# yuriyvnv/speech_transcript_embeddings

Hardware: AMD Instinct MI355X
Metric: audio–text pairs/sec (whole node), 10s@16kHz + 64-tok, 1/2/4/8 MI355X (higher is better)
Workload: dtype bf16; 1 GPU; c2: global batch 64 = 1 GPU x 1 micro-batch(es) of 64 pairs, each pair 10s@16kHz audio + 64-tok clean + 64-tok corrupt; w2v-bert-2.0 Conformer 24L + XLM-R-base 12L, 3+3 unfrozen; GPU fbank -> fwd -> InfoNCE -> bwd -> allreduce -> clip+AdamW; global_batch=64, local_batch=64, micro_batch=64, accumulation_steps=1, seq_len_audio_frames=499, seq_len_text=64, parallelism=dp1

## Files before the change

profiles/attn_probe.py:

```python
import argparse
import json
import os
import sys

import torch

sys.path.insert(0, os.path.dirname(os.path.dirname(os.path.abspath(__file__))))


def main():
    ap = argparse.ArgumentParser()
    ap.add_argument("--batch", type=int, default=64)
    ap.add_argument("--frames", type=int, default=499)
    ap.add_argument("--heads", type=int, default=16)
    ap.add_argument("--iters", type=int, default=20)
    ap.add_argument("--no-bwd", action="store_true")
    ap.add_argument("--no-split", action="store_true", help="forward without the O_lo (hi + lo P) product")
    a = ap.parse_args()
    from speech_transcript_embeddings_amd import ops
    B, T, H = a.batch, a.frames, a.heads
    D = 64 * H
    M = B * T
    g = torch.Generator(device="cuda").manual_seed(0)
    qkv = torch.randn(M, 3 * D, device="cuda", generator=g) * 0.6
    qkv[:, 2 * D:] += torch.randn(B, 1, D, device="cuda", generator=g).expand(B, T, D).reshape(M, D)
    qkv = qkv.bfloat16()
    q, k, v = qkv[:, :D], qkv[:, D:2 * D], qkv[:, 2 * D:]
    mask = torch.ones(B, T, dtype=torch.int32, device="cuda")
    for b in range(0, B, 4):
        mask[b, T - 1 - (b % 37):] = 0
    mask = mask.reshape(-1).contiguous()
    E = (torch.randn(73, 64, device="cuda", generator=g) * 0.3).bfloat16()
    o = torch.empty(M, D, device="cuda", dtype=torch.bfloat16)
    o_lo = torch.empty_like(o)
    lse = torch.empty(B * H * T, device="cuda")
    do = (torch.randn(M, D, device="cuda", generator=g)).bfloat16()
    dqkv = torch.empty(M, 3 * D, device="cuda", dtype=torch.bfloat16)
    delta = torch.empty(B * H * T, device="cuda")
    dE = torch.zeros(73, 64, device="cuda")
    gwork = torch.empty(B * H * T * 80, device="cuda")

    def fwd():
        ops.attention_fwd(q, k, v, B=B, T=T, H=H, o=o, lse=lse, key_mask=mask, rel_E=E, scale=0.125,
                          o_lo=None if a.no_split else o_lo)

    def bwd():
        ops.attention_bwd(q, k, v, o, lse, do, dqkv[:, :D], dqkv[:, D:2 * D], dqkv[:, 2 * D:], B=B, T=T, H=H,
                          delta=delta, key_mask=mask, rel_E=E, scale=0.125, dE=dE, gwork=gwork, o_lo=o_lo)

    fwd()
    if not a.no_bwd:
        bwd()
    torch.cuda.synchronize()
    res = {}
    for name, fn in (("fwd", fwd),) + (() if a.no_bwd else (("bwd", bwd),)):
        e0, e1 = torch.cuda.Event(enable_timing=True), torch.cuda.Event(enable_timing=True)
        e0.record()
        for _ in range(a.iters):
            fn()
        e1.record()
        torch.cuda.synchronize()
        res[name + "_us"] = round(e0.elapsed_time(e1) * 1e3 / a.iters, 1)
    fl = 4.0 * B * H * T * T * 64
    fl_rel = 2.0 * B * H * T * 73 * 64
    res["fwd_tflops"] = round((fl + fl_rel) / res["fwd_us"] / 1e6, 1)
    if "bwd_us" in res:
        res["bwd_tflops"] = round((2.5 * fl + 2 * fl_rel) / res["bwd_us"] / 1e6, 1)
    res["shape"] = {"B": B, "T": T, "H": H}
    print(json.dumps(res), flush=True)


if __name__ == "__main__":
    main()
```

speech_transcript_embeddings_amd/csrc/attention.hip:

```cpp
#include <type_traits>
#include "common.h"
#include "../../include/ste.h"

#ifndef STE_ABLATE
#define STE_ABLATE 0
#endif

namespace {

constexpr int HD = 64;
constexpr int TQ = 64;
constexpr int TK = 64;
constexpr int NT = 256;
constexpr int TILE = TK * HD * 2;
constexpr int NREL = 80;
constexpr float NEG_MASK = -3.4028234663852886e38f;

STE_DEV int swz(int row, int chunk) { return row * 128 + ((chunk ^ (row & 7)) << 4); }

STE_DEV int med3i(int d, int lo, int hi) {
  int r;
  asm("v_med3_i32 %0, %1, %2, %3" : "=v"(r) : "v"(d), "v"(lo), "v"(hi));
  return r;
}

STE_DEV void tile_ld(bf16x8 (&r)[2], const bf16* base, int64_t ld, int bT, int row0, int T, int tid) {
#pragma unroll
  for (int i = 0; i < 2; ++i) {
    int c = tid + NT * i, row = c >> 3, ch = c & 7;
    if (row0 + row < T) r[i] = *reinterpret_cast<const bf16x8*>(base + (int64_t)(bT + row0 + row) * ld + ch * 8);
    else r[i] = bf16x8{};
  }
}
STE_DEV void tile_st(char* t, const bf16x8 (&r)[2], int tid) {
#pragma unroll
  for (int i = 0; i < 2; ++i) {
    int c = tid + NT * i;
    *reinterpret_cast<bf16x8*>(t + swz(c >> 3, c & 7)) = r[i];
  }
}
STE_DEV bf16x8 frag_kc(const char* t, int rb, int s, int lane) {
  int r = rb + (lane & 15);
  return *reinterpret_cast<const bf16x8*>(t + swz(r, s * 4 + (lane >> 4)));
}
STE_DEV int tr_off(int row, int quad) { return row * 128 + ((((quad >> 1) ^ (row & 7))) << 4) + ((quad & 1) << 3); }
STE_DEV bf16x8 frag_tr(const char* t, int cb, int u, int lane) {
  int g = lane >> 4, li = lane & 15, q = li >> 2, p = li & 3;
  int r0 = 32 * u + 4 * g + q;
  int quad = (cb >> 2) + p;
  return join_tr(ds_read_tr16(t + tr_off(r0, quad)), ds_read_tr16(t + tr_off(r0 + 16, quad)));
}
STE_DEV bf16x8 pack_acc(f32x4 a, f32x4 b) {
  bf16x8 v;
  v[0] = (bf16)a[0]; v[1] = (bf16)a[1]; v[2] = (bf16)a[2]; v[3] = (bf16)a[3];
  v[4] = (bf16)b[0]; v[5] = (bf16)b[1]; v[6] = (bf16)b[2]; v[7] = (bf16)b[3];
  return v;
}

typedef float f32x2 __attribute__((ext_vector_type(2)));

STE_DEV bf16x8 pack_acc_lo(f32x4 a, f32x4 b, bf16x8 hi) {
  typedef unsigned u32x4 __attribute__((ext_vector_type(4)));
  const u32x4 hu = __builtin_bit_cast(u32x4, hi);
  const f32x4 x[2] = {a, b};
  bf16x8 v;
#pragma unroll
  for (int w = 0; w < 4; ++w) {
    const f32x2 h = {__builtin_bit_cast(float, hu[w] << 16), __builtin_bit_cast(float, hu[w] & 0xffff0000u)};
    const f32x2 d = f32x2{x[w >> 1][2 * (w & 1)], x[w >> 1][2 * (w & 1) + 1]} - h;
    v[2 * w] = (bf16)d[0];
    v[2 * w + 1] = (bf16)d[1];
  }
  return v;
}

STE_DEV void stage_E(char* sE, const bf16* E, int nrel, int rows, int tid) {
  for (int c = tid; c < rows * 8; c += NT) {
    int row = c >> 3, ch = c & 7;
    bf16x8 v = bf16x8{};
    if (row < nrel) v = *reinterpret_cast<const bf16x8*>(E + row * HD + ch * 8);
    *reinterpret_cast<bf16x8*>(sE + swz(row, ch)) = v;
  }
}
STE_DEV void build_qe(float* qe, const char* sE, const bf16x8 (&qf)[2], int lane) {
  const int g = lane >> 4, li = lane & 15;
#pragma unroll
  for (int jt = 0; jt < NREL / 16; ++jt) {
    f32x4 acc = {0.f, 0.f, 0.f, 0.f};
#pragma unroll
    for (int s = 0; s < 2; ++s) acc = mfma16(frag_kc(sE, jt * 16, s, lane), qf[s], acc);
#pragma unroll
    for (int r = 0; r < 4; ++r) qe[li * NREL + jt * 16 + 4 * g + r] = acc[r];
  }
}

STE_DEV float key_flag(const int32_t* mask, int bT, int key, int T) {
  if (key >= T) return -1.f;
  return (mask == nullptr || mask[bT + key] != 0) ? 1.f : 0.f;
}

STE_DEV void tile_of_block(int T, int H, int& tile, int& h, int& b) {
  const int ntile = (T + 63) / 64;
  const int id = xcd_remap(blockIdx.x, gridDim.x);
  tile = id % ntile;
  const int bh = id / ntile;
  h = bh % H;
  b = bh / H;
}

template <bool REL, bool DROP>
__global__ __launch_bounds__(NT, 2) void attn_fwd_kernel(ste_attn_args a) {
  extern __shared__ __attribute__((aligned(16))) char sm[];
  char* sK = sm;
  char* sV = sm + 2 * TILE;
  char* sE = sm + 4 * TILE;
  float* sQE = reinterpret_cast<float*>(sE + NREL * 128);
  float* sMask = sQE + 4 * 16 * NREL;

  const int tid = threadIdx.x, lane = tid & 63, w = tid >> 6, g = lane >> 4, li = lane & 15;
  int tile, h, b;
  tile_of_block(a.T, a.H, tile, h, b);
  const int T = a.T, H = a.H, bT = b * T;
  const int q0 = tile * TQ + w * 16, myq = q0 + li;
  const bf16* Qb = (const bf16*)a.q + h * HD;
  const bf16* Kb = (const bf16*)a.k + h * HD;
  const bf16* Vb = (const bf16*)a.v + h * HD;
  const int left = a.rel_left, right = a.rel_right, nrel = left + right + 1;

  bf16x8 qf[2];
#pragma unroll
  for (int s = 0; s < 2; ++s)
    qf[s] = myq < T ? *reinterpret_cast<const bf16x8*>(Qb + (int64_t)(bT + myq) * a.ldq + 32 * s + 8 * g) : bf16x8{};

  float* qe = sQE + w * 16 * NREL;
  float qe_lo = 0.f, qe_hi = 0.f;
  if (REL) {
    stage_E(sE, (const bf16*)a.rel_E, nrel, NREL, tid);
    __syncthreads();
    build_qe(qe, sE, qf, lane);
    __builtin_amdgcn_s_waitcnt(0xc07f);
    __builtin_amdgcn_wave_barrier();
    qe_lo = qe[li * NREL];
    qe_hi = qe[li * NREL + nrel - 1];
  }

  const uint32_t thresh = (uint32_t)(a.drop_p * 4294967296.0);
  const float inv_keep = DROP ? 1.0f / (1.0f - a.drop_p) : 1.0f;
  const uint64_t drow = ((uint64_t)(b * H + h) * T + myq) * (uint64_t)T;
  const bool split = a.o_lo != nullptr;

  float m = -INFINITY, l = 0.f;
  f32x4 o[4];
#pragma unroll
  for (int i = 0; i < 4; ++i) o[i] = f32x4{0.f, 0.f, 0.f, 0.f};

  const int nkt = (T + TK - 1) / TK;
  bf16x8 rk[2], rv[2];
  tile_ld(rk, Kb, a.ldk, bT, 0, T, tid);
  tile_ld(rv, Vb, a.ldv, bT, 0, T, tid);
  tile_st(sK, rk, tid);
  tile_st(sV, rv, tid);
  if (tid < 64) sMask[tid] = key_flag(a.key_mask, bT, tid, T);
  __syncthreads();

  for (int kt = 0; kt < nkt; ++kt) {
    const int cur = kt & 1, kb = kt * TK;
    const bool more = kt + 1 < nkt;
    float mk_next = 0.f;
    if (more) {
      tile_ld(rk, Kb, a.ldk, bT, kb + TK, T, tid);
      tile_ld(rv, Vb, a.ldv, bT, kb + TK, T, tid);
      if (tid < 64) mk_next = key_flag(a.key_mask, bT, kb + TK + tid, T);
    }
    const char* tK = sK + cur * TILE;
    const char* tV = sV + cur * TILE;
    const float* mk = sMask + cur * 64;

    f32x4 s[4];
#pragma unroll
    for (int t = 0; t < 4; ++t) {
      s[t] = f32x4{0.f, 0.f, 0.f, 0.f};
#pragma unroll
      for (int ss = 0; ss < 2; ++ss) s[t] = mfma16(frag_kc(tK, t * 16, ss, lane), qf[ss], s[t]);
    }
    const bool all_lo = (kb + TK - 1) - q0 <= -left;
    const bool all_hi = kb - (q0 + 15) >= right;
    float tmax = -INFINITY;
#pragma unroll
    for (int t = 0; t < 4; ++t)
#pragma unroll
      for (int r = 0; r < 4; ++r) {
        const int kl = 16 * t + 4 * g + r;
        float bias = 0.f;
        if (REL) {
          if (all_lo) bias = qe_lo;
          else if (all_hi) bias = qe_hi;
          else {
            int d = kb + kl - myq;
            d = med3i(d, -left, right);
            bias = qe[li * NREL + d + left];
          }
        }
        float v = (s[t][r] + bias) * a.scale;
        const float f = mk[kl];
        v = f > 0.5f ? v : (f < -0.5f ? -INFINITY : NEG_MASK);
        s[t][r] = v;
        tmax = fmaxf(tmax, v);
      }
    tmax = fmaxf(tmax, __shfl_xor(tmax, 16, 64));
    tmax = fmaxf(tmax, __shfl_xor(tmax, 32, 64));
    const float mnew = fmaxf(m, tmax);
    const float alpha = (mnew == -INFINITY) ? 1.f : __expf(m - mnew);
    float psum = 0.f;
#pragma unroll
    for (int t = 0; t < 4; ++t)
#pragma unroll
      for (int r = 0; r < 4; ++r) {
        float p = (mnew == -INFINITY) ? 0.f : __expf(s[t][r] - mnew);
        psum += p;
        if (DROP) p *= drop_scale(a.seed, drow + (uint64_t)(kb + 16 * t + 4 * g + r), thresh, inv_keep);
        s[t][r] = p;
      }
    psum += __shfl_xor(psum, 16, 64);
    psum += __shfl_xor(psum, 32, 64);
    l = l * alpha + psum;
    m = mnew;
#pragma unroll
    for (int dt = 0; dt < 4; ++dt) o[dt] *= alpha;
#pragma unroll
    for (int u = 0; u < 2; ++u) {
      const bf16x8 pb = pack_acc(s[2 * u], s[2 * u + 1]);
#pragma unroll
      for (int dt = 0; dt < 4; ++dt) o[dt] = mfma16(frag_tr(tV, dt * 16, u, lane), pb, o[dt]);
      if (split) {
        const bf16x8 pl = pack_acc_lo(s[2 * u], s[2 * u + 1], pb);
#pragma unroll
        for (int dt = 0; dt < 4; ++dt) o[dt] = mfma16(frag_tr(tV, dt * 16, u, lane), pl, o[dt]);
      }
    }
    if (more) {
      tile_st(sK + (cur ^ 1) * TILE, rk, tid);
      tile_st(sV + (cur ^ 1) * TILE, rv, tid);
      if (tid < 64) sMask[(cur ^ 1) * 64 + tid] = mk_next;
    }
    __syncthreads();
  }
  if (myq < T) {
    const bool zrow = a.zero_masked_rows && m == NEG_MASK;
    const float inv_l = zrow ? 0.f : 1.0f / l;
    bf16* O = (bf16*)a.o + (int64_t)(bT + myq) * a.ldo + h * HD;
    if (a.o_lo) {
      bf16* Ol = (bf16*)a.o_lo + (int64_t)(bT + myq) * a.ldolo + h * HD;
#pragma unroll
      for (int dt = 0; dt < 4; ++dt) store_bf16x4_split(O + 16 * dt + 4 * g, Ol + 16 * dt + 4 * g, o[dt] * inv_l);
    } else {
#pragma unroll
      for (int dt = 0; dt < 4; ++dt) store_bf16x4(O + 16 * dt + 4 * g, o[dt] * inv_l);
    }
    if (g == 0) a.lse[(int64_t)(b * H + h) * T + myq] = m == NEG_MASK ? (zrow ? INFINITY : -INFINITY) : m + logf(l);
  }
}
// ... 1008 lines not shown
    }
#pragma unroll
    for (int gq = 0; gq < 2; ++gq) {
      const int q0g = qw + 16 * gq, myq = q0g + li;
      float* row = tb + (16 * gq + li) * GT3 + left;
      const bool all_lo = nrel == 1 || (kb + TK - 1) - q0g <= -left;
      const bool all_hi = kb - (q0g + 15) >= right;
      const bool band = !(all_lo || all_hi);
      if (!band) {
        const float cb = all_lo ? blo[gq] : bhi[gq];
#pragma unroll
        for (int t = 0; t < 4; ++t)
#pragma unroll
          for (int r = 0; r < 4; ++r) sc[gq][t][r] = __builtin_amdgcn_exp2f(fmaf(sc[gq][t][r], c2, cb));
      } else {
#pragma unroll
        for (int t = 0; t < 4; ++t)
#pragma unroll
          for (int r = 0; r < 4; ++r) {
            int d = kb + 16 * t + 4 * g + r - myq;
            d = med3i(d, -left, right);
            sc[gq][t][r] = __builtin_amdgcn_exp2f(fmaf(sc[gq][t][r] + row[d], c2, nl2[gq]));
          }
      }
      if (!all_valid) {
#pragma unroll
        for (int t = 0; t < 4; ++t)
#pragma unroll
          for (int r = 0; r < 4; ++r) {
            const int bit = 4 * t + r;
            const float fill = ((inp >> bit) & 1u) ? pm[gq] : 0.f;
            sc[gq][t][r] = ((okp >> bit) & 1u) ? sc[gq][t][r] : fill;
          }
      }
      float bsum = 0.f;
#pragma unroll
      for (int t = 0; t < 4; ++t)
#pragma unroll
        for (int r = 0; r < 4; ++r) {
          const float ds = sc[gq][t][r] * (dp[gq][t][r] - dl[gq]);
          sc[gq][t][r] = ds;
          bsum += ds;
        }
      if (!band) {
        if (all_lo) glo[gq] += bsum; else ghi[gq] += bsum;
      } else {
        float* spare = row + (GT3 - 1 - left);
#pragma unroll
        for (int t = 0; t < 4; ++t)
#pragma unroll
          for (int r = 0; r < 4; ++r) {
            const int d = kb + 16 * t + 4 * g + r - myq;
            const bool lo = d <= -left, hi = d >= right;
            glo[gq] += lo ? sc[gq][t][r] : 0.f;
            ghi[gq] += hi ? sc[gq][t][r] : 0.f;
            *((lo || hi) ? spare : row + d) = sc[gq][t][r];
          }
      }
    }
    asm volatile("s_waitcnt lgkmcnt(0)" ::: "memory");
    __builtin_amdgcn_sched_barrier(0);
#pragma unroll
    for (int gq = 0; gq < 2; ++gq)
#pragma unroll
      for (int u = 0; u < 2; ++u) {
        const bf16x8 pb = pack_acc(sc[gq][2 * u], sc[gq][2 * u + 1]);
#pragma unroll
        for (int dt = 0; dt < 4; ++dt) dq[gq][dt] = mfma16(ktr[dt][u], pb, dq[gq][dt]);
      }
    if (kt + 1 < nkt) {
      asm volatile("s_waitcnt vmcnt(0)" ::: "memory");
      __builtin_amdgcn_s_barrier();
      if (kt + 2 < nkt) issue(kt + 2);
    }
  }
  if (nkt > 1) issue_E(sm + (nkt & 1) * KV);
  const int kend = nkt * TK;
#pragma unroll
  for (int gq = 0; gq < 2; ++gq) {
    glo[gq] = rowsum4(glo[gq]);
    ghi[gq] = rowsum4(ghi[gq]);
    const int myq = qw + 16 * gq + li;
    float* row = tb + (16 * gq + li) * GT3;
    for (int j = 1 + g; j < nrel - 1; j += 4) {
      const int k = myq + j - left;
      if (k < 0 || k >= kend) row[j] = 0.f;
    }
    if (g == 1) row[GT3 - 1] = 0.f;
    if (g == 0) {
      row[0] = glo[gq];
      if (nrel > 1) row[nrel - 1] = ghi[gq];
    }
  }
  asm volatile("s_waitcnt vmcnt(0)" ::: "memory");
  __syncthreads();
  const char* sE = sm + (nkt & 1) * KV;
#pragma unroll
  for (int gq = 0; gq < 2; ++gq) {
    const float* row = tb + (16 * gq + li) * GT3;
#pragma unroll
    for (int u = 0; u < 2; ++u) {
      const f32x4 g0 = *reinterpret_cast<const f32x4*>(row + 32 * u + 4 * g);
      const f32x4 g1 = *reinterpret_cast<const f32x4*>(row + 32 * u + 16 + 4 * g);
      const bf16x8 pb = pack_acc(g0, g1);
#pragma unroll
      for (int dt = 0; dt < 4; ++dt) dq[gq][dt] = mfma16(frag_tr(sE, dt * 16, u, lane), pb, dq[gq][dt]);
    }
    const f32x4 gt4 = *reinterpret_cast<const f32x4*>(row + 64 + 4 * g);
    bf16x4 gb;
    gb[0] = (bf16)gt4[0]; gb[1] = (bf16)gt4[1]; gb[2] = (bf16)gt4[2]; gb[3] = (bf16)gt4[3];
    const int q = li >> 2, pq = li & 3;
#pragma unroll
    for (int dt = 0; dt < 4; ++dt) {
      const s16x4 ea = ds_read_tr16(sE + tr_off(64 + 4 * g + q, dt * 4 + pq));
      dq[gq][dt] = __builtin_amdgcn_mfma_f32_16x16x16bf16_1k(ea, __builtin_bit_cast(s16x4, gb), dq[gq][dt], 0, 0, 0);
    }
  }
#pragma unroll
  for (int gq = 0; gq < 2; ++gq) {
    const int myq = qw + 16 * gq + li;
    if (myq >= T) continue;
    const int64_t rowid = (int64_t)(b * H + h) * T + myq;
    const float* row = tb + (16 * gq + li) * GT3;
    if (a.dE) {
      float* G = a.gwork + rowid * NREL;
#pragma unroll
      for (int c = 0; c < NREL / 16; ++c) {
        const int j = c * 16 + 4 * g;
        *reinterpret_cast<f32x4*>(G + j) = *reinterpret_cast<const f32x4*>(row + j);
      }
    }
    bf16* dQ = (bf16*)a.dq + (int64_t)(bT + myq) * a.lddq + h * HD;
#pragma unroll
    for (int dt = 0; dt < 4; ++dt) store_bf16x4(dQ + 16 * dt + 4 * g, dq[gq][dt] * a.scale);
  }
}

namespace rel2 {
constexpr int KB = 128;
constexpr int QD = 2 * TILE + 512;
constexpr int KV_E_OFF = 2 * QD;
constexpr int KV_QE_OFF = KV_E_OFF + NREL * 128;
constexpr int QE3 = NREL + 4;
constexpr int KV_EDGE3_OFF = KV_QE_OFF + 64 * QE3 * 4;
constexpr int DKV3_LDS = KV_EDGE3_OFF + 512;
}

__global__ __launch_bounds__(NT, 2) void attn_bwd_dkv_rel3_kernel(ste_attn_args a) {
  using namespace rel2;
  extern __shared__ __attribute__((aligned(16))) char sm[];
  const int tid = threadIdx.x, lane = tid & 63, g = lane >> 4, li = lane & 15;
  const int w = __builtin_amdgcn_readfirstlane(tid >> 6);
  const int T = a.T, H = a.H;
  const int ntile = (T + KB - 1) / KB;
  const int id = xcd_remap(blockIdx.x, gridDim.x);
  const int tile = id % ntile, bh = id / ntile, h = bh % H, b = bh / H, bT = b * T;
  const int left = a.rel_left, right = a.rel_right, nrel = left + right + 1;
  const bf16* Qb = (const bf16*)a.q + h * HD;
  const bf16* Kb = (const bf16*)a.k + h * HD;
  const bf16* Vb = (const bf16*)a.v + h * HD;
  const bf16* dOb = (const bf16*)a.dout + h * HD;
  const int kb0 = tile * KB, k0w = kb0 + w * 32;
  const int64_t rowbase = (int64_t)(b * H + h) * T;
  const float c2 = a.scale * LOG2E;

  bf16x8 kf[2][2], vf[2][2];
  bool kmask[2];
#pragma unroll
  for (int gk = 0; gk < 2; ++gk) {
    const int key = k0w + 16 * gk + li;
    const bool kv = key < T;
    kmask[gk] = kv && a.key_mask != nullptr && a.key_mask[bT + key] == 0;
#pragma unroll
    for (int s = 0; s < 2; ++s) {
      kf[gk][s] = kv ? *reinterpret_cast<const bf16x8*>(Kb + (int64_t)(bT + key) * a.ldk + 32 * s + 8 * g) : bf16x8{};
      vf[gk][s] = kv ? *reinterpret_cast<const bf16x8*>(Vb + (int64_t)(bT + key) * a.ldv + 32 * s + 8 * g) : bf16x8{};
    }
  }
  const bool any_masked = __ballot(kmask[0] || kmask[1]) != 0;
  char* sE = sm + KV_E_OFF;
  float* qet3 = reinterpret_cast<float*>(sm + KV_QE_OFF);
  float* elo = reinterpret_cast<float*>(sm + KV_EDGE3_OFF);
  float* ehi = elo + 64;
  stage_E(sE, (const bf16*)a.rel_E, nrel, NREL, tid);

  const int nqt = (T + TQ - 1) / TQ;
  auto issue = [&](int qt) {
    char* buf = sm + (qt & 1) * QD;
    const int qb = qt * TQ;
    glds_tile_piece32(Qb, a.ldq, bT, qb, T, buf, 2 * w);
    glds_tile_piece32(Qb, a.ldq, bT, qb, T, buf, 2 * w + 1);
    glds_tile_piece32(dOb, a.lddo, bT, qb, T, buf + TILE, 2 * w);
    glds_tile_piece32(dOb, a.lddo, bT, qb, T, buf + TILE, 2 * w + 1);
    if (w < 2) {
      const char* base = (const char*)(w == 0 ? a.lse : a.delta);
      const uint32_t off = (uint32_t)(rowbase + min(qb + lane_now(), T - 1)) * 4u;
      __builtin_amdgcn_global_load_lds((const void*)(base + off), (lds_void*)(buf + 2 * TILE + w * 256), 4, 0, 0);
    }
  };
  issue(0);
  if (nqt > 1) issue(1);
  if (nqt > 1) {
    if (w < 2) asm volatile("s_waitcnt vmcnt(5)" ::: "memory");
    else asm volatile("s_waitcnt vmcnt(4)" ::: "memory");
  } else {
    asm volatile("s_waitcnt vmcnt(0)" ::: "memory");
  }
  __syncthreads();

  f32x4 dk[2][4], dv[2][4];
#pragma unroll
  for (int gk = 0; gk < 2; ++gk)
#pragma unroll
    for (int i = 0; i < 4; ++i) {
      dk[gk][i] = f32x4{0.f, 0.f, 0.f, 0.f};
      dv[gk][i] = dk[gk][i];
    }

  for (int qt = 0; qt < nqt; ++qt) {
    const char* tQ = sm + (qt & 1) * QD;
    const char* tD = tQ + TILE;
    const float* sL = reinterpret_cast<const float*>(tQ + 2 * TILE);
    const int qb = qt * TQ;
    const bool blk_lo = (kb0 + KB - 1) - qb <= -left;
    const bool blk_hi = kb0 - (qb + TQ - 1) >= right;
    const bool blk_band = !(blk_lo || blk_hi);
    {
      bf16x8 qfr[2];
#pragma unroll
      for (int s = 0; s < 2; ++s) qfr[s] = frag_kc(tQ, 16 * w, s, lane);
      float* qrow = qet3 + (16 * w + li) * QE3;
#pragma unroll
      for (int jt = 0; jt < NREL / 16; ++jt) {
        if (!blk_band && jt != 0 && jt != (nrel - 1) / 16) continue;
        f32x4 acc = {0.f, 0.f, 0.f, 0.f};
#pragma unroll
        for (int s = 0; s < 2; ++s) acc = mfma16(frag_kc(sE, jt * 16, s, lane), qfr[s], acc);
        *reinterpret_cast<f32x4*>(qrow + jt * 16 + 4 * g) = acc;
      }
      if (g == 0) {
        const int l16 = lane_now() & 15;
        const float nl = sL[16 * w + l16] * -LOG2E;
        elo[16 * w + l16] = qrow[0] * c2 + nl;
        ehi[16 * w + l16] = qrow[nrel - 1] * c2 + nl;
      }
    }
    __syncthreads();
#pragma unroll
    for (int u = 0; u < 2; ++u) {
      f32x4 sc[2][2], dp[2][2];
      f32x4 lsev[2], ndl[2];
#pragma unroll
      for (int nn = 0; nn < 2; ++nn) {
        lsev[nn] = *reinterpret_cast<const f32x4*>(sL + 16 * (2 * u + nn) + 4 * g);
        ndl[nn] = -*reinterpret_cast<const f32x4*>(sL + 64 + 16 * (2 * u + nn) + 4 * g);
      }
#pragma unroll
      for (int nn = 0; nn < 2; ++nn) {
        const int n = 2 * u + nn;
        bf16x8 qa[2], da[2];
#pragma unroll
        for (int ss = 0; ss < 2; ++ss) {
          qa[ss] = frag_kc(tQ, 16 * n, ss, lane);
          da[ss] = frag_kc(tD, 16 * n, ss, lane);
        }
#pragma unroll
        for (int gk = 0; gk < 2; ++gk) {
          sc[gk][nn] = mfma16(qa[0], kf[gk][0], f32x4{0.f, 0.f, 0.f, 0.f});
          dp[gk][nn] = mfma16(da[0], vf[gk][0], ndl[nn]);
          sc[gk][nn] = mfma16(qa[1], kf[gk][1], sc[gk][nn]);
          dp[gk][nn] = mfma16(da[1], vf[gk][1], dp[gk][nn]);
        }
      }
      bf16x8 trd[4], trq[4];
#pragma unroll
      for (int dt = 0; dt < 4; ++dt) {
        trd[dt] = frag_tr_asm(tD, dt * 16, u, lane);
        trq[dt] = frag_tr_asm(tQ, dt * 16, u, lane);
      }
      bf16x8 pv[2], pk[2];
#pragma unroll
      for (int gk = 0; gk < 2; ++gk) {
        const int k0g = k0w + 16 * gk, mykey = k0g + li;
        const bool all_lo = (k0g + 15) - qb <= -left;
        const bool all_hi = k0g - (qb + TQ - 1) >= right;
#pragma unroll
        for (int nn = 0; nn < 2; ++nn) {
          const int n = 2 * u + nn;
          if (all_lo || all_hi) {
            const f32x4 eb = *reinterpret_cast<const f32x4*>((all_lo ? elo : ehi) + 16 * n + 4 * g);
#pragma unroll
            for (int r = 0; r < 4; ++r) sc[gk][nn][r] = __builtin_amdgcn_exp2f(fmaf(sc[gk][nn][r], c2, eb[r]));
          } else {
            const f32x4 nl2 = lsev[nn] * -LOG2E;
#pragma unroll
            for (int r = 0; r < 4; ++r) {
              const int ql = 16 * n + 4 * g + r;
              int d = mykey - (qb + ql);
              d = med3i(d, -left, right);
              sc[gk][nn][r] = __builtin_amdgcn_exp2f(fmaf(sc[gk][nn][r] + qet3[ql * QE3 + d + left], c2, nl2[r]));
            }
          }
          if (any_masked && kmask[gk]) {
#pragma unroll
            for (int r = 0; r < 4; ++r) sc[gk][nn][r] = lsev[nn][r] == -INFINITY ? 1.0f / T : 0.f;
          }
          if (qb + TQ > T) {
#pragma unroll
            for (int r = 0; r < 4; ++r)
              if (qb + 16 * n + 4 * g + r >= T) sc[gk][nn][r] = 0.f;
          }
          dp[gk][nn] = sc[gk][nn] * dp[gk][nn];
        }
        pv[gk] = pack_acc(sc[gk][0], sc[gk][1]);
        pk[gk] = pack_acc(dp[gk][0], dp[gk][1]);
      }
      asm volatile("s_waitcnt lgkmcnt(0)" ::: "memory");
      __builtin_amdgcn_sched_barrier(0);
#pragma unroll
      for (int dt = 0; dt < 4; ++dt) {
#pragma unroll
        for (int gk = 0; gk < 2; ++gk) {
          dv[gk][dt] = mfma16(trd[dt], pv[gk], dv[gk][dt]);
          dk[gk][dt] = mfma16(trq[dt], pk[gk], dk[gk][dt]);
        }
      }
    }
    if (qt + 1 < nqt) {
      asm volatile("s_waitcnt vmcnt(0)" ::: "memory");
      __builtin_amdgcn_s_barrier();
      if (qt + 2 < nqt) issue(qt + 2);
    }
  }
#pragma unroll
  for (int gk = 0; gk < 2; ++gk) {
    const int key = k0w + 16 * gk + li;
    if (key < T) {
      bf16* dK = (bf16*)a.dk + (int64_t)(bT + key) * a.lddk + h * HD;
      bf16* dV = (bf16*)a.dv + (int64_t)(bT + key) * a.lddv + h * HD;
#pragma unroll
      for (int dt = 0; dt < 4; ++dt) {
        store_bf16x4(dK + 16 * dt + 4 * g, dk[gk][dt] * a.scale);
        store_bf16x4(dV + 16 * dt + 4 * g, dv[gk][dt]);
      }
    }
  }
}

__global__ __launch_bounds__(256) void attn_rel_dE2_kernel(ste_attn_args a) {
  __shared__ float sG[64][16];
  __shared__ float sQ[64][HD];
  const int tid = threadIdx.x;
  const int T = a.T, nbh = a.B * a.H;
  const int nrel = a.rel_left + a.rel_right + 1;
  const int j0 = 16 * blockIdx.x, jr = tid >> 4, d0 = (tid & 15) * 4;
  f32x4 acc = f32x4{0.f, 0.f, 0.f, 0.f};
  for (int bh = 0; bh < nbh; ++bh) {
    const int h = bh % a.H, b = bh / a.H;
    const float* G = a.gwork + (int64_t)bh * T * NREL + j0;
    const bf16* Q = (const bf16*)a.q + (int64_t)b * T * a.ldq + h * HD;
    for (int t0 = 0; t0 < T; t0 += 64) {
      const int nr = min(64, T - t0);
      __syncthreads();
      {
        const int r = tid >> 2, c = (tid & 3) * 4;
        const f32x4 v = r < nr ? *reinterpret_cast<const f32x4*>(G + (int64_t)(t0 + r) * NREL + c) : f32x4{0.f, 0.f, 0.f, 0.f};
        *reinterpret_cast<f32x4*>(&sG[r][c]) = v;
      }
      for (int i = tid; i < 64 * (HD / 8); i += 256) {
        const int r = i / (HD / 8), c = (i % (HD / 8)) * 8;
        const bf16x8 v = r < nr ? *reinterpret_cast<const bf16x8*>(Q + (int64_t)(t0 + r) * a.ldq + c) : bf16x8{};
#pragma unroll
        for (int e = 0; e < 8; ++e) sQ[r][c + e] = (float)v[e];
      }
      __syncthreads();
      for (int r = 0; r < nr; ++r) acc += *reinterpret_cast<const f32x4*>(&sQ[r][d0]) * sG[r][jr];
    }
  }
  const int j = j0 + jr;
  if (j < nrel) {
    f32x4* o = reinterpret_cast<f32x4*>(a.dE + j * HD + d0);
    *o = *o + acc * a.scale;
  }
}

namespace rel_de {
constexpr int IMG = TILE;
constexpr int LDS = 5 * IMG;
constexpr int MIN_T = 64;
}

__global__ __launch_bounds__(256) void attn_rel_dE3_kernel(ste_attn_args a) {
  using namespace rel_de;
  extern __shared__ __attribute__((aligned(16))) char sm[];
  const int tid = threadIdx.x, lane = tid & 63, g = lane >> 4, li = lane & 15;
  const int w = __builtin_amdgcn_readfirstlane(tid >> 6);
  const int bh = blockIdx.x, h = bh % a.H, b = bh / a.H, T = a.T;
  float* G = a.gwork + (int64_t)bh * T * NREL;
  const bf16* Q = (const bf16*)a.q + (int64_t)b * T * a.ldq + h * HD;
  char* const qi = sm + 4 * IMG;
  f32x4 acc[5];
#pragma unroll
  for (int jt = 0; jt < 5; ++jt) acc[jt] = f32x4{0.f, 0.f, 0.f, 0.f};
  f32x4 gv[5];
  bf16x8 qv[2];
  auto load = [&](int t0) {
#pragma unroll
    for (int k = 0; k < 5; ++k) {
      const int i = tid + 256 * k, r = i / 20, c = (i % 20) * 4;
      gv[k] = t0 + r < T ? *reinterpret_cast<const f32x4*>(G + (int64_t)(t0 + r) * NREL + c) : f32x4{0.f, 0.f, 0.f, 0.f};
    }
#pragma unroll
    for (int k = 0; k < 2; ++k) {
      const int i = tid + 256 * k, r = i >> 3, c = (i & 7) * 8;
      qv[k] = t0 + r < T ? *reinterpret_cast<const bf16x8*>(Q + (int64_t)(t0 + r) * a.ldq + c) : bf16x8{};
    }
  };
  const int nch = (T + 63) / 64;
  load(0);
  for (int ch = 0; ch < nch; ++ch) {
    __syncthreads();
#pragma unroll
    for (int k = 0; k < 5; ++k) {
      const int i = tid + 256 * k, r = i / 20, c = (i % 20) * 4;
      bf16x4 hi, lo;
#pragma unroll
      for (int e = 0; e < 4; ++e) {
        hi[e] = (bf16)gv[k][e];
        lo[e] = (bf16)(gv[k][e] - (float)hi[e]);
      }
      const int off = tr_off(r, (c & 63) >> 2);
      *reinterpret_cast<bf16x4*>(sm + (c >> 6) * IMG + off) = hi;
      *reinterpret_cast<bf16x4*>(sm + (2 + (c >> 6)) * IMG + off) = lo;
    }
#pragma unroll
    for (int k = 0; k < 2; ++k) {
      const int i = tid + 256 * k, r = i >> 3, c = (i & 7) * 8;
      *reinterpret_cast<bf16x8*>(qi + tr_off(r, c >> 2)) = qv[k];
    }
    if (ch + 1 < nch) load((ch + 1) * 64);
    __syncthreads();
#pragma unroll
    for (int u = 0; u < 2; ++u) {
      const bf16x8 qb = frag_tr(qi, 16 * w, u, lane);
#pragma unroll
      for (int jt = 0; jt < 5; ++jt) {
        acc[jt] = mfma16(frag_tr(sm + (jt >> 2) * IMG, (jt & 3) * 16, u, lane), qb, acc[jt]);
        acc[jt] = mfma16(frag_tr(sm + (2 + (jt >> 2)) * IMG, (jt & 3) * 16, u, lane), qb, acc[jt]);
      }
    }
  }
  __syncthreads();
#pragma unroll
  for (int jt = 0; jt < 5; ++jt)
#pragma unroll
    for (int r = 0; r < 4; ++r) G[(16 * jt + 4 * g + r) * HD + 16 * w + li] = acc[jt][r];
}

__global__ __launch_bounds__(1024) void attn_rel_dE3_sum_kernel(ste_attn_args a) {
  __shared__ float red[16][HD];
  const int j = blockIdx.x, d = threadIdx.x & 63, sub = threadIdx.x >> 6;
  const int nbh = a.B * a.H;
  const int64_t stride = (int64_t)a.T * NREL;
  const float* P = a.gwork + j * HD + d;
  float s = 0.f;
  int p = sub;
  for (; p + 48 < nbh; p += 64) {
    const float v0 = P[p * stride], v1 = P[(p + 16) * stride], v2 = P[(p + 32) * stride], v3 = P[(p + 48) * stride];
    s += v0; s += v1; s += v2; s += v3;
  }
  for (; p < nbh; p += 16) s += P[p * stride];
  red[sub][d] = s;
  __syncthreads();
  if (sub == 0) {
    float t = 0.f;
#pragma unroll
    for (int k = 0; k < 16; ++k) t += red[k][d];
    a.dE[j * HD + d] += t * a.scale;
  }
}

constexpr int FWD_LDS = 4 * TILE + NREL * 128 + 4 * 16 * NREL * 4 + 2 * 64 * 4;
constexpr int DQ_LDS = 2 * TILE + 96 * 128 + 4 * 16 * NREL * 4 + 4 * 16 * 96 * 4 + 64 * 4;
constexpr int DKV_LDS = 4 * TILE + NREL * 128 + 64 * NREL * 4 + 2 * 128 * 4;

bool ab_is(const char* name, char v) {
  const char* e = STE_AB_ENV(name);
  return e && e[0] == v;
}
bool rel_de3() {
  static const bool v = !ab_is("STE_ATTN_DE", '2');
  return v;
}
bool rel_fwd_v4() {
  static const bool v = !ab_is("STE_ATTN_FWD", '2');
  return v;
}
bool rel_fwd_plo() {
  static const bool v = !ab_is("STE_ATTN_PLO", '0');
  return v;
}

int check(const ste_attn_args* a) {
  if (!a || a->B <= 0 || a->T <= 0 || a->H <= 0) return STE_ERR_ARG;
  if ((a->ldq & 7) || (a->ldk & 7) || (a->ldv & 7) || (a->ldo & 7)) return STE_ERR_SHAPE;
  if (a->o_lo && (a->ldolo & 7)) return STE_ERR_SHAPE;
  if (a->rel_E && a->rel_left + a->rel_right + 1 > NREL) return STE_ERR_SHAPE;
  if (a->drop_p < 0.f || a->drop_p >= 1.f) return STE_ERR_ARG;
  if (a->rel_E && a->zero_masked_rows) return STE_ERR_ARG;
  return 0;
}

int launch_dE(const ste_attn_args* a, hipStream_t s) {
  const int nrel = a->rel_left + a->rel_right + 1;
  if (a->T >= rel_de::MIN_T && rel_de3()) {
    hipLaunchKernelGGL(attn_rel_dE3_kernel, dim3((unsigned)(a->B * a->H)), dim3(256), rel_de::LDS, s, *a);
    STE_CHECK_LAUNCH();
    hipLaunchKernelGGL(attn_rel_dE3_sum_kernel, dim3((unsigned)nrel), dim3(1024), 0, s, *a);
  } else {
    hipLaunchKernelGGL(attn_rel_dE2_kernel, dim3((unsigned)((nrel + 15) / 16)), dim3(256), 0, s, *a);
  }
  STE_CHECK_LAUNCH();
  return 0;
}

}

extern "C" int ste_attention_fwd(const ste_attn_args* a, void* stream) {
  if (int e = check(a)) return e;
  if (!a->lse || !a->o) return STE_ERR_ARG;
  hipStream_t s = (hipStream_t)stream;
  dim3 grid((unsigned)(((a->T + TQ - 1) / TQ) * a->H * a->B));
  const bool rel = a->rel_E != nullptr, drop = a->drop_p > 0.f;
  if (rel && !drop) {
    dim3 g2((unsigned)(((a->T + rel2::BQ - 1) / rel2::BQ) * a->H * a->B));
    if (rel_fwd_v4() && a->rel_left + a->rel_right + 1 <= rel4::max_nrel() && a->T <= rel4::MAXT * TK) {
      if (a->o_lo && rel_fwd_plo()) hipLaunchKernelGGL((attn_fwd_rel4_kernel<true, true>), g2, dim3(NT), rel4::FWD_LDS, s, *a);
      else if (a->o_lo) hipLaunchKernelGGL((attn_fwd_rel4_kernel<true, false>), g2, dim3(NT), rel4::FWD_LDS, s, *a);
      else hipLaunchKernelGGL((attn_fwd_rel4_kernel<false, false>), g2, dim3(NT), rel4::FWD_LDS, s, *a);
    } else if (a->o_lo)
      hipLaunchKernelGGL(attn_fwd_rel2_kernel<true>, g2, dim3(NT), rel2::FWD_LDS, s, *a);
    else
      hipLaunchKernelGGL(attn_fwd_rel2_kernel<false>, g2, dim3(NT), rel2::FWD_LDS, s, *a);
    STE_CHECK_LAUNCH();
    return 0;
  }
  if (rel && drop) hipLaunchKernelGGL((attn_fwd_kernel<true, true>), grid, dim3(NT), FWD_LDS, s, *a);
  else if (rel) hipLaunchKernelGGL((attn_fwd_kernel<true, false>), grid, dim3(NT), FWD_LDS, s, *a);
  else if (drop) hipLaunchKernelGGL((attn_fwd_kernel<false, true>), grid, dim3(NT), FWD_LDS, s, *a);
  else hipLaunchKernelGGL((attn_fwd_kernel<false, false>), grid, dim3(NT), FWD_LDS, s, *a);
  STE_CHECK_LAUNCH();
  return 0;
}

extern "C" int ste_attention_bwd(const ste_attn_args* a, void* stream) {
  if (int e = check(a)) return e;
  if (!a->dout || !a->o || !a->lse || !a->delta || !a->dq || !a->dk || !a->dv) return STE_ERR_ARG;
  if ((a->lddo & 7) || (a->lddq & 3) || (a->lddk & 3) || (a->lddv & 3)) return STE_ERR_SHAPE;
  if (a->dE && (!a->gwork || !a->rel_E)) return STE_ERR_ARG;
  hipStream_t s = (hipStream_t)stream;
  if (a->rel_E && a->drop_p == 0.f) {
    static_assert(NREL < rel2::GT3, "bin GT3-1 is the dQ kernel's spare slot");
    dim3 gq((unsigned)(((a->T + rel2::DQ3_Q - 1) / rel2::DQ3_Q) * a->H * a->B));
    hipLaunchKernelGGL(attn_bwd_dq_rel3_kernel, gq, dim3(NT), rel2::DQ3_LDS, s, *a);
    STE_CHECK_LAUNCH();
    dim3 gk((unsigned)(((a->T + rel2::KB - 1) / rel2::KB) * a->H * a->B));
    hipLaunchKernelGGL(attn_bwd_dkv_rel3_kernel, gk, dim3(NT), rel2::DKV3_LDS, s, *a);
    STE_CHECK_LAUNCH();
    if (a->dE) return launch_dE(a, s);
    return 0;
  }
  hipLaunchKernelGGL(attn_delta_kernel, dim3((unsigned)(((int64_t)a->B * a->T + 3) / 4)), dim3(256), 0, s, *a);
  STE_CHECK_LAUNCH();
  dim3 grid((unsigned)(((a->T + TQ - 1) / TQ) * a->H * a->B));
  const bool rel = a->rel_E != nullptr, drop = a->drop_p > 0.f;
#define STE_LAUNCH2(KER, LDS)                                                            \
  if (rel && drop) hipLaunchKernelGGL((KER<true, true>), grid, dim3(NT), LDS, s, *a);    \
  else if (rel) hipLaunchKernelGGL((KER<true, false>), grid, dim3(NT), LDS, s, *a);      \
  else if (drop) hipLaunchKernelGGL((KER<false, true>), grid, dim3(NT), LDS, s, *a);     \
  else hipLaunchKernelGGL((KER<false, false>), grid, dim3(NT), LDS, s, *a);              \
  STE_CHECK_LAUNCH();
  STE_LAUNCH2(attn_bwd_dq_kernel, DQ_LDS)
  STE_LAUNCH2(attn_bwd_dkv_kernel, DKV_LDS)
#undef STE_LAUNCH2
  if (a->dE) return launch_dE(a, s);
  return 0;
}
```

Baseline: 488.7 pairs/s.

## Process two key tiles per block in rel-bias dK/dV backward kernel

```diff
diff --git a/profiles/attn_probe.py b/profiles/attn_probe.py
--- a/profiles/attn_probe.py
+++ b/profiles/attn_probe.py
@@ -16,6 +16,8 @@
     ap.add_argument("--iters", type=int, default=20)
     ap.add_argument("--no-bwd", action="store_true")
     ap.add_argument("--no-split", action="store_true", help="forward without the O_lo (hi + lo P) product")
+    ap.add_argument("--left", type=int, default=64, help="distance window; --left 0 --right 0 is one bin: no band tiles")
+    ap.add_argument("--right", type=int, default=8)
     a = ap.parse_args()
     from speech_transcript_embeddings_amd import ops
     B, T, H = a.batch, a.frames, a.heads
@@ -30,7 +32,8 @@
     for b in range(0, B, 4):
         mask[b, T - 1 - (b % 37):] = 0
     mask = mask.reshape(-1).contiguous()
-    E = (torch.randn(73, 64, device="cuda", generator=g) * 0.3).bfloat16()
+    nrel = a.left + a.right + 1
+    E = (torch.randn(73, 64, device="cuda", generator=g) * 0.3).bfloat16()[:nrel].contiguous()
     o = torch.empty(M, D, device="cuda", dtype=torch.bfloat16)
     o_lo = torch.empty_like(o)
     lse = torch.empty(B * H * T, device="cuda")
@@ -42,11 +45,12 @@
 
     def fwd():
         ops.attention_fwd(q, k, v, B=B, T=T, H=H, o=o, lse=lse, key_mask=mask, rel_E=E, scale=0.125,
-                          o_lo=None if a.no_split else o_lo)
+                          rel_left=a.left, rel_right=a.right, o_lo=None if a.no_split else o_lo)
 
     def bwd():
         ops.attention_bwd(q, k, v, o, lse, do, dqkv[:, :D], dqkv[:, D:2 * D], dqkv[:, 2 * D:], B=B, T=T, H=H,
-                          delta=delta, key_mask=mask, rel_E=E, scale=0.125, dE=dE, gwork=gwork, o_lo=o_lo)
+                          delta=delta, key_mask=mask, rel_E=E, rel_left=a.left, rel_right=a.right, scale=0.125, dE=dE,
+                          gwork=gwork, o_lo=o_lo)
 
     fwd()
     if not a.no_bwd:
@@ -66,7 +70,7 @@
     res["fwd_tflops"] = round((fl + fl_rel) / res["fwd_us"] / 1e6, 1)
     if "bwd_us" in res:
         res["bwd_tflops"] = round((2.5 * fl + 2 * fl_rel) / res["bwd_us"] / 1e6, 1)
-    res["shape"] = {"B": B, "T": T, "H": H}
+    res["shape"] = {"B": B, "T": T, "H": H, "left": a.left, "right": a.right}
     print(json.dumps(res), flush=True)
 
 
diff --git a/profiles/compare_dumps.py b/profiles/compare_dumps.py
--- /dev/null
+++ b/profiles/compare_dumps.py
@@ -0,0 +1,33 @@
+import sys
+from pathlib import Path
+
+import numpy as np
+
+
+def main(a, b):
+    names = sorted({p.name for p in Path(a).glob("*.npy")} | {p.name for p in Path(b).glob("*.npy")})
+    bad = not names
+    for n in names:
+        pa, pb = Path(a) / n, Path(b) / n
+        if not (pa.exists() and pb.exists()):
+            print(f"{n}: missing on one side")
+            bad = True
+            continue
+        x, y = np.load(pa), np.load(pb)
+        same = x.shape == y.shape and x.dtype == y.dtype and np.array_equal(
+            np.ascontiguousarray(x).view(np.uint8), np.ascontiguousarray(y).view(np.uint8))
+        if same:
+            print(f"{n}: {x.dtype} {tuple(x.shape)} equal bit for bit")
+        else:
+            bad = True
+            if x.shape == y.shape:
+                d = x != y
+                print(f"{n}: {tuple(x.shape)} DIFFERS in {int(d.sum())} entries, max |a - b| "
+                      f"{float(np.abs(x.astype(np.float64) - y.astype(np.float64)).max()):.3e}")
+            else:
+                print(f"{n}: shapes differ {x.shape} vs {y.shape}")
+    return 1 if bad else 0
+
+
+if __name__ == "__main__":
+    sys.exit(main(sys.argv[1], sys.argv[2]))
diff --git a/speech_transcript_embeddings_amd/csrc/attention.hip b/speech_transcript_embeddings_amd/csrc/attention.hip
--- a/speech_transcript_embeddings_amd/csrc/attention.hip
+++ b/speech_transcript_embeddings_amd/csrc/attention.hip
@@ -107,6 +107,8 @@
   h = bh % H;
   b = bh / H;
 }
+
+STE_HD int pair_count(int ntile) { return (ntile + 1) / 2; }
 
 template <bool REL, bool DROP>
 __global__ __launch_bounds__(NT, 2) void attn_fwd_kernel(ste_attn_args a) {
@@ -1421,32 +1423,35 @@
   const int tid = threadIdx.x, lane = tid & 63, g = lane >> 4, li = lane & 15;
   const int w = __builtin_amdgcn_readfirstlane(tid >> 6);
   const int T = a.T, H = a.H;
-  const int ntile = (T + KB - 1) / KB;
+  const int ntile = (T + KB - 1) / KB, npair = pair_count(ntile);
   const int id = xcd_remap(blockIdx.x, gridDim.x);
-  const int tile = id % ntile, bh = id / ntile, h = bh % H, b = bh / H, bT = b * T;
+  const int tile0 = 2 * (id % npair), bh = id / npair, h = bh % H, b = bh / H, bT = b * T;
+  const int ntl = min(2, ntile - tile0);
   const int left = a.rel_left, right = a.rel_right, nrel = left + right + 1;
   const bf16* Qb = (const bf16*)a.q + h * HD;
   const bf16* Kb = (const bf16*)a.k + h * HD;
   const bf16* Vb = (const bf16*)a.v + h * HD;
   const bf16* dOb = (const bf16*)a.dout + h * HD;
-  const int kb0 = tile * KB, k0w = kb0 + w * 32;
   const int64_t rowbase = (int64_t)(b * H + h) * T;
   const float c2 = a.scale * LOG2E;
 
   bf16x8 kf[2][2], vf[2][2];
   bool kmask[2];
-#pragma unroll
-  for (int gk = 0; gk < 2; ++gk) {
-    const int key = k0w + 16 * gk + li;
-    const bool kv = key < T;
-    kmask[gk] = kv && a.key_mask != nullptr && a.key_mask[bT + key] == 0;
-#pragma unroll
-    for (int s = 0; s < 2; ++s) {
-      kf[gk][s] = kv ? *reinterpret_cast<const bf16x8*>(Kb + (int64_t)(bT + key) * a.ldk + 32 * s + 8 * g) : bf16x8{};
-      vf[gk][s] = kv ? *reinterpret_cast<const bf16x8*>(Vb + (int64_t)(bT + key) * a.ldv + 32 * s + 8 * g) : bf16x8{};
-    }
-  }
-  const bool any_masked = __ballot(kmask[0] || kmask[1]) != 0;
+  auto load_keys = [&](int k0w_) {
+#pragma unroll
+    for (int gk = 0; gk < 2; ++gk) {
+      const int key = k0w_ + 16 * gk + li;
+      const bool kv = key < T;
+      kmask[gk] = kv && a.key_mask != nullptr && a.key_mask[bT + key] == 0;
+#pragma unroll
+      for (int s = 0; s < 2; ++s) {
+        kf[gk][s] = kv ? *reinterpret_cast<const bf16x8*>(Kb + (int64_t)(bT + key) * a.ldk + 32 * s + 8 * g) : bf16x8{};
+        vf[gk][s] = kv ? *reinterpret_cast<const bf16x8*>(Vb + (int64_t)(bT + key) * a.ldv + 32 * s + 8 * g) : bf16x8{};
+      }
+    }
+  };
+  load_keys(tile0 * KB + w * 32);
+  bool any_masked = __ballot(kmask[0] || kmask[1]) != 0;
   char* sE = sm + KV_E_OFF;
   float* qet3 = reinterpret_cast<float*>(sm + KV_QE_OFF);
   float* elo = reinterpret_cast<float*>(sm + KV_EDGE3_OFF);
@@ -1469,149 +1474,163 @@
   };
   issue(0);
   if (nqt > 1) issue(1);
-  if (nqt > 1) {
-    if (w < 2) asm volatile("s_waitcnt vmcnt(5)" ::: "memory");
-    else asm volatile("s_waitcnt vmcnt(4)" ::: "memory");
-  } else {
-    asm volatile("s_waitcnt vmcnt(0)" ::: "memory");
-  }
-  __syncthreads();
-
-  f32x4 dk[2][4], dv[2][4];
-#pragma unroll
-  for (int gk = 0; gk < 2; ++gk)
-#pragma unroll
-    for (int i = 0; i < 4; ++i) {
-      dk[gk][i] = f32x4{0.f, 0.f, 0.f, 0.f};
-      dv[gk][i] = dk[gk][i];
-    }
-
-  for (int qt = 0; qt < nqt; ++qt) {
-    const char* tQ = sm + (qt & 1) * QD;
-    const char* tD = tQ + TILE;
-    const float* sL = reinterpret_cast<const float*>(tQ + 2 * TILE);
-    const int qb = qt * TQ;
-    const bool blk_lo = (kb0 + KB - 1) - qb <= -left;
-    const bool blk_hi = kb0 - (qb + TQ - 1) >= right;
-    const bool blk_band = !(blk_lo || blk_hi);
-    {
-      bf16x8 qfr[2];
-#pragma unroll
-      for (int s = 0; s < 2; ++s) qfr[s] = frag_kc(tQ, 16 * w, s, lane);
-      float* qrow = qet3 + (16 * w + li) * QE3;
-#pragma unroll
-      for (int jt = 0; jt < NREL / 16; ++jt) {
-        if (!blk_band && jt != 0 && jt != (nrel - 1) / 16) continue;
-        f32x4 acc = {0.f, 0.f, 0.f, 0.f};
-#pragma unroll
-        for (int s = 0; s < 2; ++s) acc = mfma16(frag_kc(sE, jt * 16, s, lane), qfr[s], acc);
-        *reinterpret_cast<f32x4*>(qrow + jt * 16 + 4 * g) = acc;
-      }
-      if (g == 0) {
-        const int l16 = lane_now() & 15;
-        const float nl = sL[16 * w + l16] * -LOG2E;
-        elo[16 * w + l16] = qrow[0] * c2 + nl;
-        ehi[16 * w + l16] = qrow[nrel - 1] * c2 + nl;
-      }
+
+  for (int tl = 0; tl < ntl; ++tl) {
+    const int kb0 = (tile0 + tl) * KB, k0w = kb0 + w * 32;
+    if (nqt > 1) {
+      if (w < 2) asm volatile("s_waitcnt vmcnt(5)" ::: "memory");
+      else asm volatile("s_waitcnt vmcnt(4)" ::: "memory");
+    } else {
+      asm volatile("s_waitcnt vmcnt(0)" ::: "memory");
     }
     __syncthreads();
-#pragma unroll
-    for (int u = 0; u < 2; ++u) {
-      f32x4 sc[2][2], dp[2][2];
-      f32x4 lsev[2], ndl[2];
-#pragma unroll
-      for (int nn = 0; nn < 2; ++nn) {
-        lsev[nn] = *reinterpret_cast<const f32x4*>(sL + 16 * (2 * u + nn) + 4 * g);
-        ndl[nn] = -*reinterpret_cast<const f32x4*>(sL + 64 + 16 * (2 * u + nn) + 4 * g);
-      }
-#pragma unroll
-      for (int nn = 0; nn < 2; ++nn) {
-        const int n = 2 * u + nn;
-        bf16x8 qa[2], da[2];
-#pragma unroll
-        for (int ss = 0; ss < 2; ++ss) {
-          qa[ss] = frag_kc(tQ, 16 * n, ss, lane);
-          da[ss] = frag_kc(tD, 16 * n, ss, lane);
+
+    f32x4 dk[2][4], dv[2][4];
+#pragma unroll
+    for (int gk = 0; gk < 2; ++gk)
+#pragma unroll
+      for (int i = 0; i < 4; ++i) {
+        dk[gk][i] = f32x4{0.f, 0.f, 0.f, 0.f};
+        dv[gk][i] = dk[gk][i];
+      }
+
+    for (int qt = 0; qt < nqt; ++qt) {
+      const char* tQ = sm + (qt & 1) * QD;
+      const char* tD = tQ + TILE;
+      const float* sL = reinterpret_cast<const float*>(tQ + 2 * TILE);
+      const int qb = qt * TQ;
+      const bool blk_lo = (kb0 + KB - 1) - qb <= -left;
+      const bool blk_hi = kb0 - (qb + TQ - 1) >= right;
+      const bool blk_band = !(blk_lo || blk_hi);
+      {
+        bf16x8 qfr[2];
+#pragma unroll
+        for (int s = 0; s < 2; ++s) qfr[s] = frag_kc(tQ, 16 * w, s, lane);
+        float* qrow = qet3 + (16 * w + li) * QE3;
+#pragma unroll
+        for (int jt = 0; jt < NREL / 16; ++jt) {
+          if (!blk_band && jt != 0 && jt != (nrel - 1) / 16) continue;
+          f32x4 acc = {0.f, 0.f, 0.f, 0.f};
+#pragma unroll
+          for (int s = 0; s < 2; ++s) acc = mfma16(frag_kc(sE, jt * 16, s, lane), qfr[s], acc);
+          *reinterpret_cast<f32x4*>(qrow + jt * 16 + 4 * g) = acc;
         }
-#pragma unroll
-        for (int gk = 0; gk < 2; ++gk) {
-          sc[gk][nn] = mfma16(qa[0], kf[gk][0], f32x4{0.f, 0.f, 0.f, 0.f});
-          dp[gk][nn] = mfma16(da[0], vf[gk][0], ndl[nn]);
-          sc[gk][nn] = mfma16(qa[1], kf[gk][1], sc[gk][nn]);
-          dp[gk][nn] = mfma16(da[1], vf[gk][1], dp[gk][nn]);
+        if (g == 0) {
+          const int l16 = lane_now() & 15;
+          const float nl = sL[16 * w + l16] * -LOG2E;
+          elo[16 * w + l16] = qrow[0] * c2 + nl;
+          ehi[16 * w + l16] = qrow[nrel - 1] * c2 + nl;
         }
       }
-      bf16x8 trd[4], trq[4];
-#pragma unroll
-      for (int dt = 0; dt < 4; ++dt) {
-        trd[dt] = frag_tr_asm(tD, dt * 16, u, lane);
-        trq[dt] = frag_tr_asm(tQ, dt * 16, u, lane);
-      }
-      bf16x8 pv[2], pk[2];
-#pragma unroll
-      for (int gk = 0; gk < 2; ++gk) {
-        const int k0g = k0w + 16 * gk, mykey = k0g + li;
-        const bool all_lo = (k0g + 15) - qb <= -left;
-        const bool all_hi = k0g - (qb + TQ - 1) >= right;
+      __syncthreads();
+#pragma unroll
+      for (int u = 0; u < 2; ++u) {
+        f32x4 sc[2][2], dp[2][2];
+        f32x4 lsev[2], ndl[2];
+#pragma unroll
+        for (int nn = 0; nn < 2; ++nn) {
+          lsev[nn] = *reinterpret_cast<const f32x4*>(sL + 16 * (2 * u + nn) + 4 * g);
+          ndl[nn] = -*reinterpret_cast<const f32x4*>(sL + 64 + 16 * (2 * u + nn) + 4 * g);
+        }
 #pragma unroll
         for (int nn = 0; nn < 2; ++nn) {
           const int n = 2 * u + nn;
-          if (all_lo || all_hi) {
-            const f32x4 eb = *reinterpret_cast<const f32x4*>((all_lo ? elo : ehi) + 16 * n + 4 * g);
-#pragma unroll
-            for (int r = 0; r < 4; ++r) sc[gk][nn][r] = __builtin_amdgcn_exp2f(fmaf(sc[gk][nn][r], c2, eb[r]));
-          } else {
-            const f32x4 nl2 = lsev[nn] * -LOG2E;
-#pragma unroll
-            for (int r = 0; r < 4; ++r) {
-              const int ql = 16 * n + 4 * g + r;
-              int d = mykey - (qb + ql);
-              d = med3i(d, -left, right);
-              sc[gk][nn][r] = __builtin_amdgcn_exp2f(fmaf(sc[gk][nn][r] + qet3[ql * QE3 + d + left], c2, nl2[r]));
+          bf16x8 qa[2], da[2];
+#pragma unroll
+          for (int ss = 0; ss < 2; ++ss) {
+            qa[ss] = frag_kc(tQ, 16 * n, ss, lane);
+            da[ss] = frag_kc(tD, 16 * n, ss, lane);
+          }
+#pragma unroll
+          for (int gk = 0; gk < 2; ++gk) {
+            sc[gk][nn] = mfma16(qa[0], kf[gk][0], f32x4{0.f, 0.f, 0.f, 0.f});
+            dp[gk][nn] = mfma16(da[0], vf[gk][0], ndl[nn]);
+            sc[gk][nn] = mfma16(qa[1], kf[gk][1], sc[gk][nn]);
+            dp[gk][nn] = mfma16(da[1], vf[gk][1], dp[gk][nn]);
+          }
+        }
+        bf16x8 trd[4], trq[4];
+#pragma unroll
+        for (int dt = 0; dt < 4; ++dt) {
+          trd[dt] = frag_tr_asm(tD, dt * 16, u, lane);
+          trq[dt] = frag_tr_asm(tQ, dt * 16, u, lane);
+        }
+        bf16x8 pv[2], pk[2];
+#pragma unroll
+        for (int gk = 0; gk < 2; ++gk) {
+          const int k0g = k0w + 16 * gk, mykey = k0g + li;
+          const bool all_lo = (k0g + 15) - qb <= -left;
+          const bool all_hi = k0g - (qb + TQ - 1) >= right;
+#pragma unroll
+          for (int nn = 0; nn < 2; ++nn) {
+            const int n = 2 * u + nn;
+            if (all_lo || all_hi) {
+              const f32x4 eb = *reinterpret_cast<const f32x4*>((all_lo ? elo : ehi) + 16 * n + 4 * g);
+#pragma unroll
+              for (int r = 0; r < 4; ++r) sc[gk][nn][r] = __builtin_amdgcn_exp2f(fmaf(sc[gk][nn][r], c2, eb[r]));
+            } else {
+              const f32x4 nl2 = lsev[nn] * -LOG2E;
+#pragma unroll
+              for (int r = 0; r < 4; ++r) {
+                const int ql = 16 * n + 4 * g + r;
+                int d = mykey - (qb + ql);
+                d = med3i(d, -left, right);
+                sc[gk][nn][r] = __builtin_amdgcn_exp2f(fmaf(sc[gk][nn][r] + qet3[ql * QE3 + d + left], c2, nl2[r]));
+              }
             }
+            if (any_masked && kmask[gk]) {
+#pragma unroll
+              for (int r = 0; r < 4; ++r) sc[gk][nn][r] = lsev[nn][r] == -INFINITY ? 1.0f / T : 0.f;
+            }
+            if (qb + TQ > T) {
+#pragma unroll
+              for (int r = 0; r < 4; ++r)
+                if (qb + 16 * n + 4 * g + r >= T) sc[gk][nn][r] = 0.f;
+            }
+            dp[gk][nn] = sc[gk][nn] * dp[gk][nn];
           }
-          if (any_masked && kmask[gk]) {
-#pragma unroll
-            for (int r = 0; r < 4; ++r) sc[gk][nn][r] = lsev[nn][r] == -INFINITY ? 1.0f / T : 0.f;
+          pv[gk] = pack_acc(sc[gk][0], sc[gk][1]);
+          pk[gk] = pack_acc(dp[gk][0], dp[gk][1]);
+        }
+        asm volatile("s_waitcnt lgkmcnt(0)" ::: "memory");
+        __builtin_amdgcn_sched_barrier(0);
+#pragma unroll
+        for (int dt = 0; dt < 4; ++dt) {
+#pragma unroll
+          for (int gk = 0; gk < 2; ++gk) {
+            dv[gk][dt] = mfma16(trd[dt], pv[gk], dv[gk][dt]);
+            dk[gk][dt] = mfma16(trq[dt], pk[gk], dk[gk][dt]);
           }
-          if (qb + TQ > T) {
-#pragma unroll
-            for (int r = 0; r < 4; ++r)
-              if (qb + 16 * n + 4 * g + r >= T) sc[gk][nn][r] = 0.f;
-          }
-          dp[gk][nn] = sc[gk][nn] * dp[gk][nn];
         }
-        pv[gk] = pack_acc(sc[gk][0], sc[gk][1]);
-        pk[gk] = pack_acc(dp[gk][0], dp[gk][1]);
-      }
-      asm volatile("s_waitcnt lgkmcnt(0)" ::: "memory");
-      __builtin_amdgcn_sched_barrier(0);
-#pragma unroll
-      for (int dt = 0; dt < 4; ++dt) {
-#pragma unroll
-        for (int gk = 0; gk < 2; ++gk) {
-          dv[gk][dt] = mfma16(trd[dt], pv[gk], dv[gk][dt]);
-          dk[gk][dt] = mfma16(trq[dt], pk[gk], dk[gk][dt]);
+      }
+      if (qt + 1 < nqt) {
+        asm volatile("s_waitcnt vmcnt(0)" ::: "memory");
+        __builtin_amdgcn_s_barrier();
+        if (qt + 2 < nqt) issue(qt + 2);
+      }
+    }
+    const bool more = tl + 1 < ntl;
+    if (more) {
+      load_keys(k0w + KB);
+      __syncthreads();
+      issue(0);
+    }
+#pragma unroll
+    for (int gk = 0; gk < 2; ++gk) {
+      const int key = k0w + 16 * gk + li;
+      if (key < T) {
+        bf16* dK = (bf16*)a.dk + (int64_t)(bT + key) * a.lddk + h * HD;
+        bf16* dV = (bf16*)a.dv + (int64_t)(bT + key) * a.lddv + h * HD;
+#pragma unroll
+        for (int dt = 0; dt < 4; ++dt) {
+          store_bf16x4(dK + 16 * dt + 4 * g, dk[gk][dt] * a.scale);
+          store_bf16x4(dV + 16 * dt + 4 * g, dv[gk][dt]);
         }
       }
     }
-    if (qt + 1 < nqt) {
-      asm volatile("s_waitcnt vmcnt(0)" ::: "memory");
-      __builtin_amdgcn_s_barrier();
-      if (qt + 2 < nqt) issue(qt + 2);
-    }
-  }
-#pragma unroll
-  for (int gk = 0; gk < 2; ++gk) {
-    const int key = k0w + 16 * gk + li;
-    if (key < T) {
-      bf16* dK = (bf16*)a.dk + (int64_t)(bT + key) * a.lddk + h * HD;
-      bf16* dV = (bf16*)a.dv + (int64_t)(bT + key) * a.lddv + h * HD;
-#pragma unroll
-      for (int dt = 0; dt < 4; ++dt) {
-        store_bf16x4(dK + 16 * dt + 4 * g, dk[gk][dt] * a.scale);
-        store_bf16x4(dV + 16 * dt + 4 * g, dv[gk][dt]);
-      }
+    if (more) {
+      any_masked = __ballot(kmask[0] || kmask[1]) != 0;
+      issue(1);
     }
   }
 }
@@ -1833,7 +1852,7 @@
     dim3 gq((unsigned)(((a->T + rel2::DQ3_Q - 1) / rel2::DQ3_Q) * a->H * a->B));
     hipLaunchKernelGGL(attn_bwd_dq_rel3_kernel, gq, dim3(NT), rel2::DQ3_LDS, s, *a);
     STE_CHECK_LAUNCH();
-    dim3 gk((unsigned)(((a->T + rel2::KB - 1) / rel2::KB) * a->H * a->B));
+    dim3 gk((unsigned)(pair_count((a->T + rel2::KB - 1) / rel2::KB) * a->H * a->B));
     hipLaunchKernelGGL(attn_bwd_dkv_rel3_kernel, gk, dim3(NT), rel2::DKV3_LDS, s, *a);
     STE_CHECK_LAUNCH();
     if (a->dE) return launch_dE(a, s);
```

After: 488.6 pairs/s. About the same (-0.0%).
